# ViennaRNA/RNAcode

Measured on AMD Instinct MI355X. Metric: alignment-columns x samples scored /sec, higher is better.
Workload: dtype f32; 1 GPU; synthetic MAF 10000 blocks x 120 cols x 6 seqs, n=1000 (BASELINE configs[2]/[3]); exchange=none, fit_exp_mode=fused

## Files before the change

### rnacode_amd/csrc/rc_context.cpp

```cpp
#include <cstddef>

#include "rc_runtime.h"

extern "C" {

const char *rc_last_error(void) { return g_err.c_str(); }

void rc_default_params(rc_params *p) {
  p->Delta = -10.0f; p->Omega = -4.0f; p->omega = -2.0f;
  p->stopPenalty_0 = -9999.0f; p->stopPenalty_k = -8.0f;
  p->blosum = 62; p->sampleN = 100; p->cutoff = 1.0f; p->stopEarly = 0; p->seed_base = 42;
  std::memset(p->genetic_code, 0, sizeof p->genetic_code);
}

}

void want_hw_queues() { (void)setenv("GPU_MAX_HW_QUEUES", "8", 0); }

int table_set(rc_ctx *c, const rc_params &par, const TableSet **out) {
  char code[64];
  const char *why = nullptr;
  if (!parse_genetic_code(par.genetic_code, code, &why)) return fail(RC_ERR_ARG, why);
  if (par.blosum != 62 && par.blosum != 90) return fail(RC_ERR_ARG, "blosum must be 62 or 90");
  std::lock_guard<std::mutex> lk(c->setMutex);
// ... 37 lines not shown
  c->sets.push_back(std::move(t));
  return RC_OK;
}

extern "C" {

int rc_device_count(void) {
  want_hw_queues();
  int n = 0;
  if (hipGetDeviceCount(&n) != hipSuccess) return 0;
  return n;
}

int rc_host_cpus(void) { return effective_cpus(); }

void rc_ctx_trim(rc_ctx *c) {
  if (!c) return;
  (void)hipSetDevice(c->device);
  (void)hipDeviceSynchronize();
  c->retired->drain();
  c->bufPool->drain(false);
}

void rc_ctx_destroy(rc_ctx *c) {
  if (!c) return;
  (void)hipSetDevice(c->device);
  (void)hipDeviceSynchronize();
  c->retired->ctxGone.store(true);
  c->retired->drain();
  g_retired.drain();
  c->bufPool->drain(true);
  c->pool.reset();
  if (kProfiling && c->d_cellStats.p) {
    unsigned long long st[8] = {0, 0, 0, 0, 0, 0, 0, 0};
    if (hipMemcpy(st, c->d_cellStats.p, sizeof st, hipMemcpyDeviceToHost) == hipSuccess && st[0])
      std::fprintf(stderr, "[rc cell stats] wavefront-cells %llu, with no positive lane %llu (%.4f %%), positive lane-cells %.2f %%\n", st[0], st[1],
                   100.0 * st[1] / st[0], 100.0 * st[2] / (64.0 * st[0])),
      std::fprintf(stderr, "[rc cell stats] before the row's first event %.1f %%, event codons %.1f %%, after its last event %.1f %%, between events %.1f %%\n",
                   100.0 * st[3] / st[0], 100.0 * st[4] / st[0], 100.0 * st[5] / st[0], 100.0 * (st[0] - st[3] - st[4] - st[5]) / st[0]),
      std::fprintf(stderr, "[rc cell stats] buffered row: chunks tested against the scan's gate %llu, passed over %llu (%.2f %%)\n", st[6], st[7],
                   st[6] ? 100.0 * st[7] / st[6] : 0.0);
  }
  if (c->d_U) (void)hipFree(c->d_U);
  for (hipStream_t st : c->compute) if (st) (void)hipStreamDestroy(st);
  if (c->native) (void)hipStreamDestroy(c->native);
  if (c->copy) (void)hipStreamDestroy(c->copy);
  if (c->aux) (void)hipStreamDestroy(c->aux);
  if (c->tree) (void)hipStreamDestroy(c->tree);
  if (c->tree2) (void)hipStreamDestroy(c->tree2);
  for (hipStream_t st : c->classStreams) (void)hipStreamDestroy(st);
  delete c;
}

int rc_ctx_create(int device, rc_ctx **out) {
  if (!out) return fail(RC_ERR_ARG, "null out pointer");
  *out = nullptr;
  want_hw_queues();
  int n = 0;
  trace("ctx: start", nullptr);
  if (hipGetDeviceCount(&n) != hipSuccess || n <= 0)
    return fail(RC_ERR_DEVICE, "no HIP device available: the scoring path has no CPU fallback");
  trace("ctx: runtime up", nullptr);
  if (device < 0 || device >= n) return fail(RC_ERR_ARG, "device index out of range");
  HIP_TRY(hipSetDevice(device));
  std::unique_ptr<rc_ctx, void (*)(rc_ctx *)> guard(new rc_ctx(), rc_ctx_destroy);
  rc_ctx *c = guard.get();
  c->device = device;
  hipDeviceProp_t prop;
  HIP_TRY(hipGetDeviceProperties(&prop, device));
  c->numCU = prop.multiProcessorCount;
  c->totalMem = prop.totalGlobalMem;
  c->retiredCapBytes = prop.totalGlobalMem / 16;
  c->bufPool->devCap = prop.totalGlobalMem / 16;
  c->bufPool->device = device;
// ... 20 lines not shown
  if (const char *e = std::getenv("RC_DUAL_ROWS")) c->dualRows = std::atoi(e) != 0;
  if (const char *e = std::getenv("RC_HIGH_OCCUPANCY")) c->highOccupancy = std::max(0, std::min(2, std::atoi(e)));
  if (prop.maxSharedMemoryPerMultiProcessor > 0) c->ldsPerCU = prop.maxSharedMemoryPerMultiProcessor;
  if (const char *e = std::getenv("RC_FAT_STREAM_MIN_ITEMS")) c->fatStreamMinItems = std::max(0ll, std::atoll(e));
  if (const char *e = std::getenv("RC_GENERIC_SCRATCH_MB")) c->genericScratchWords = std::max<size_t>(1, static_cast<size_t>(std::atoll(e))) * (1u << 20) / sizeof(uint32_t);
  int prioLow = 0, prioHigh = 0;
  HIP_TRY(hipDeviceGetStreamPriorityRange(&prioLow, &prioHigh));
  c->prioLow = prioLow; c->prioHigh = 0; c->classPrio = prioLow;
  trace("ctx: streams", nullptr);
  c->serialNative = std::getenv("RC_SERIAL_NATIVE") ? 1 : 0;
  c->stopTwoRoundsMinItems = 4LL * c->numCU * 16;
  if (const char *e = std::getenv("RC_STOP_MIN_ITEMS")) c->stopTwoRoundsMinItems = std::atoll(e);
  if (const char *e = std::getenv("RC_GENERIC_MIN_ROWS")) c->rule.genericMinRows = std::max(3, std::min(kTemplRows + 1, std::atoi(e)));
  if (const char *e = std::getenv("RC_TILED_MAX_L")) c->rule.tiledMaxL = std::max(0, std::atoi(e));
  if (const char *e = std::getenv("RC_TILED_MIN_ROWS")) c->rule.tiledMinRows = std::max(kTiledMaxKT + 2, std::min(kTemplRows + 1, std::atoi(e)));
  if (const char *e = std::getenv("RC_TILED_MAX_ROWS")) c->rule.tiledMaxRows = std::max(kTemplRows, std::min(kMaxRows, std::atoi(e)));
  if (const char *e = std::getenv("RC_TILED_WIDE_MAX_L")) c->rule.tiledWideMaxL = std::max(0, std::atoi(e));
  if (const char *e = std::getenv("RC_TILED_ANY_L_MIN_ROWS")) c->rule.tiledAnyLMinRows = std::max(kTemplRows + 1, std::atoi(e));
  if (const char *e = std::getenv("RC_STOP_ROUNDS")) c->stopRounds = std::max(2, std::min(kMaxRounds, std::atoi(e)));
  {
    rc_params std{};
    std.blosum = 62;
    const TableSet *unused = nullptr;
    RC_TRY(table_set(c, std, &unused));
    std.blosum = 90;
    RC_TRY(table_set(c, std, &unused));
  }
  trace("ctx: tables", nullptr);
  c->tieThr = float_threshold_lt(0.0001);
  if (const char *e = std::getenv("RC_LDS_MAX_BYTES")) { c->ldsMaxBytes = c->ldsMaxBytesOneRow = static_cast<size_t>(std::atol(e)); c->stageManyRows = true; }
#ifdef RC_PROFILING
  if (const char *e = std::getenv("RC_DEBUG_SKIP")) c->debugSkip = std::atoi(e);
  if (std::getenv("RC_CELL_STATS")) {
    HIP_TRY(c->d_cellStats.ensure(8 * sizeof(unsigned long long)));
    HIP_TRY(hipMemset(c->d_cellStats.p, 0, 8 * sizeof(unsigned long long)));
  }
#endif
  c->hostThreads = std::min(effective_cpus(), 32);
  if (const char *e = std::getenv("RC_HOST_THREADS")) c->hostThreads = std::max(1, std::atoi(e));
  *out = guard.release();
  return RC_OK;
}

int rc_genetic_code(int32_t ncbi_id, char out[65]) {
  if (!out) return fail(RC_ERR_ARG, "null out pointer");
  const char *aas = ncbi_code(ncbi_id);
  if (!aas) return fail(RC_ERR_ARG, "unknown genetic code id " + std::to_string(ncbi_id) +
                                    " (built in: 1-6, 9-14, 16, 21-26, 29, 30, 33; 27, 28, 31 and 32 are not supported)");
  std::memcpy(out, aas, 64);
  out[64] = '\0';
  return RC_OK;
}

int rc_ctx_set_host_threads(rc_ctx *c, int32_t threads) {
  if (!c || threads < 1) return fail(RC_ERR_ARG, "bad argument");
  if (c->inflight.load() != 0) return fail(RC_ERR_ARG, "batches are in flight");
  c->hostThreads = threads;
  c->pool.reset();
  return RC_OK;
}

int rc_ctx_host_threads(const rc_ctx *c) { return c ? c->hostThreads : 0; }

int rc_ctx_fit_exp_mode(const rc_ctx *c) { return c ? c->expMode : RC_ERR_ARG; }

}

#undef rc_default_params
// ... 33 lines not shown
```

### rnacode_amd/csrc/rc_null_kernel.h

```cpp
#pragma once
#include <hip/hip_runtime.h>

#include <type_traits>
#include <utility>

#include "rc_device.h"
#include "rc_launch.h"
#include "rc_scan_core.h"
#include "rc_sim_core.h"

namespace rc {


template <bool SEM> __device__ __forceinline__ float ref_max(float x, float y) {
  if constexpr (SEM) return x > y ? x : y;
  else return fmaxf(x, y);
}
template <bool SEM> __device__ __forceinline__ float ref_max3(float x, float y, float z) { return ref_max<SEM>(ref_max<SEM>(x, y), z); }

template <bool SEM = false>
__device__ __forceinline__ void pair_step(int zc, float sig, float Delta, float Omega, float omega,
                                          float &s0, float &s1, float &s2) {
  if (zc == 0) {
    s0 = s0 + sig;
// ... 37 lines not shown
      const float v = (j < sites) ? rows[static_cast<size_t>(a - aLo) * sites + j] : 0.0f;
      const bool last = (a == sites - 1) && (j == sites - 1);
      unsigned long long m = __ballot((j < sites) && (v > 0.0f || last));
      while (m) {
        const int t = __builtin_ctzll(m);
        m &= m - 1ull;
        const int jj = j0 + t;
        const float vt = __int_as_float(__builtin_amdgcn_readlane(__float_as_int(v), t));
        scan_step(st, vt, a, jj, (a == sites - 1) && (jj == sites - 1), tieThr, [&](const ScanState &e) {
          if (out && lane == 0 && n < hssCap) out[n] = DevHss{s, f, e.ss, e.se, e.cm};
          n++;
        });
      }
    }
  }
}


template <int K> struct KReg { float s0, s1, s2; int lut; };
template <typename Seq> struct KRegs;
template <int... K> struct KRegs<std::integer_sequence<int, K...>> : KReg<K>... {
  template <int I> __device__ __forceinline__ KReg<I> &at() { return static_cast<KReg<I> &>(*this); }
};
template <int NK, typename F, int... K>
__device__ __forceinline__ void static_for_impl(F &&f, std::integer_sequence<int, K...>) {
  (f(std::integral_constant<int, K>{}), ...);
}
template <int NK, typename F> __device__ __forceinline__ void static_for(F &&f) {
  static_for_impl<NK>(static_cast<F &&>(f), std::make_integer_sequence<int, NK>{});
}

template <int NK, bool EXACT> __device__ __forceinline__ float div_by_nk(float x, float nkf) {
  if constexpr ((NK & (NK - 1)) == 0) {
    return x * (1.0f / static_cast<float>(NK));
  } else if constexpr (EXACT) {
    return x / nkf;
  } else {
    constexpr float y = 1.0f / static_cast<float>(NK);
    const float q0 = x * y;
    const float r = __builtin_fmaf(-static_cast<float>(NK), q0, x);
    return __builtin_fmaf(r, y, q0);
  }
}


struct DeepFetch {};
template <int OFF> struct StagedSite { uint32_t at; };
template <typename T> struct IsStagedSite : std::false_type {};
template <int OFF> struct IsStagedSite<StagedSite<OFF>> : std::true_type {};
template <int OFF> constexpr int staged_off(StagedSite<OFF>) { return OFF; }
__device__ __forceinline__ int site_index(int j) { return j; }
template <int OFF> __device__ __forceinline__ int site_index(StagedSite<OFF>) { return 0; }

template <int NK, bool LDSC, bool EXACT, bool DUAL, int MODE = 0>
__device__ __forceinline__ void null_body(const NullArgs &A, const uint8_t *__restrict__ blob,
                                          const DevBlock *__restrict__ dblocks, const int *__restrict__ classBlocks,
                                          const uint32_t *__restrict__ flags, const uint32_t *__restrict__ Ustream, const uint8_t *__restrict__ pairTab,
                                          uint32_t *__restrict__ scratch, float *__restrict__ maxima) {
  constexpr int N = NK + 1;
  constexpr int CPW = 5;
  constexpr int NCW = (NK + CPW - 1) / CPW;
  constexpr bool kTableLookups = !LDSC && !EXACT;
  constexpr int kTableWords = kTableLookups ? NK * kWave : 0;
  constexpr int LB = code_tail_bytes(NK);
  constexpr int PSW = code_pos_words(NK);
  using TailT = std::conditional_t<LB == 1, uint8_t, std::conditional_t<LB == 2, uint16_t, uint32_t>>;
  constexpr int ZW = (NK + 31) / 32;
  using Regs = KRegs<std::make_integer_sequence<int, NK>>;
  static_assert(!DUAL || (!EXACT && NK <= kDualRowsMaxNK), "two rows per pass: fast division, few sequences");
  static_assert(!(LDSC && EXACT), "the EXACT instantiation uses no LDS");
  constexpr bool ROWS = MODE == 1, SIM = MODE == 2;
#ifndef RC_DEEP_FETCH_MAX_NK
#define RC_DEEP_FETCH_MAX_NK 31
#endif
// ... 333 lines not shown
                  }
                }
                if (w < NCW - 1) {
                  store_words(std::integral_constant<int, 4>{}, laneWord, wf, wr, siteF + w * kWave * 4, siteR + w * kWave * 4);
                } else {
                  store_words(std::integral_constant<int, LB>{}, laneTailB, wf, wr, siteF + (NCW - 1) * kWave * 4, siteR + (NCW - 1) * kWave * 4);
                }
              }
            }
          }
        }
      }
      if (clamped && (kLean ? lane == 0 : sidx < A.sampleN) && (SIM || onlyCombo <= 0)) atomicAdd(A.clampCount, static_cast<unsigned long long>(clamped));
    }
    if constexpr (SIM) continue;
    if (!helping && shared) {
      const size_t G = gridDim.x;
      if (lane == 0) {
        __hip_atomic_store(A.steal + kStealHdr + G + 2 * blockIdx.x, static_cast<unsigned int>(bi), __ATOMIC_RELAXED, __HIP_MEMORY_SCOPE_AGENT);
        __hip_atomic_store(A.steal + kStealHdr + G + 2 * blockIdx.x + 1, static_cast<unsigned int>(grp), __ATOMIC_RELAXED, __HIP_MEMORY_SCOPE_AGENT);
      }
      __builtin_amdgcn_fence(__ATOMIC_RELEASE, "agent");
      __builtin_amdgcn_s_waitcnt(0);
      if (lane == 0) {
        atomicExch(A.steal + kStealHdr + blockIdx.x, 1u);
        const unsigned int idx = atomicAdd(A.steal, 1u);
        __hip_atomic_store(A.steal + kStealHdr + 3 * G + idx, (blockIdx.x + 1u) | (static_cast<unsigned int>(home) << 24), __ATOMIC_RELAXED, __HIP_MEMORY_SCOPE_AGENT);
        atomicSub(A.steal + 1, 1u);
      }
      firstCombo = claim_part(slot);
    }

    float best = -1.0f;
    unsigned long long statCells = 0, statNoPos = 0, statPosLanes = 0, statPristine = 0, statEvent = 0, statTail = 0, statGateTested = 0, statGateSkipped = 0;
    float omega_v, Delta_v = 0.0f;
    asm volatile("v_mov_b32 %0, %1" : "=v"(omega_v) : "s"(omega));
    float rcpNk_v = 0.0f, negNk_v = 0.0f;
    if constexpr (!EXACT && (NK & (NK - 1)) != 0) {
      asm volatile("v_mov_b32 %0, %1" : "=v"(rcpNk_v) : "s"(1.0f / static_cast<float>(NK)));
      asm volatile("v_mov_b32 %0, %1" : "=v"(negNk_v) : "s"(-static_cast<float>(NK)));
    }
    if constexpr (EXACT) asm volatile("v_mov_b32 %0, %1" : "=v"(Delta_v) : "s"(Delta));
    if (!kProfiling || !(A.debugSkip & 1)) {
      Regs R;
      int curS = -1;
      for (int c = onlyCombo >= 0 ? onlyCombo : firstCombo; c < 6; c = onlyCombo >= 0 ? 6 : (shared ? claim_part(slot) : c + 1)) {
        const int s = c >= 3 ? 1 : 0, f = c - 3 * s;
        if (s != curS) {
          static_for<NK>([&](auto kc) {
            constexpr int k = decltype(kc)::value;
            R.template at<k>().lut = __float_as_int(lut[(s * NK + k) * kLutSize + lane]);
            if constexpr (kTableLookups) lds_codes[k * kWave + lane] = static_cast<uint32_t>(R.template at<k>().lut);
          });
          curS = s;
        }
        const int sites = (L - f) / 3;
        if (sites <= 0) continue;
        const uint32_t *__restrict__ sbase = cod + static_cast<size_t>(s * L1 + 3 + f) * PSW;
        constexpr int kSiteWords = 3 * PSW;
        auto word_at = [&](int j, int x) -> uint32_t {
          const uint32_t *p = sbase + static_cast<size_t>(j) * kSiteWords;
          if (x < NCW - 1) return p[x * kWave + lane];
          return static_cast<uint32_t>(reinterpret_cast<const TailT *>(p + (NCW - 1) * kWave)[lane]);
        };
        const unsigned long long *__restrict__ zbase = zw + static_cast<size_t>(s * L1 + 3 + f) * ZW;
        const unsigned long long *__restrict__ zany = zmask + static_cast<size_t>(s * 3 + f) * zmWords;
        int jc = sites;
// ... 122 lines not shown
          auto wait_lookups = [&](auto leave) {
            constexpr int k0 = (NCW - 1) * CPW;
            constexpr int cnt = NK - k0;
            constexpr int left = (decltype(leave)::value > 0 && !decltype(scalarLoadsNearby)::value) ? decltype(leave)::value : 0;
            if constexpr (cnt == 1) asm volatile("s_waitcnt lgkmcnt(%1)" : "+v"(sig[k0]) : "n"(left));
            else if constexpr (cnt == 2) asm volatile("s_waitcnt lgkmcnt(%2)" : "+v"(sig[k0]), "+v"(sig[k0 + 1]) : "n"(left));
            else if constexpr (cnt == 3) asm volatile("s_waitcnt lgkmcnt(%3)" : "+v"(sig[k0]), "+v"(sig[k0 + 1]), "+v"(sig[k0 + 2]) : "n"(left));
            else if constexpr (cnt == 4)
              asm volatile("s_waitcnt lgkmcnt(%4)" : "+v"(sig[k0]), "+v"(sig[k0 + 1]), "+v"(sig[k0 + 2]), "+v"(sig[k0 + 3]) : "n"(left));
            else
              asm volatile("s_waitcnt lgkmcnt(%5)" : "+v"(sig[k0]), "+v"(sig[k0 + 1]), "+v"(sig[k0 + 2]), "+v"(sig[k0 + 3]), "+v"(sig[k0 + 4]) : "n"(left));
            static_for<NK>([&](auto kc) {
              constexpr int k = decltype(kc)::value;
              if constexpr (k < k0) {
                float b = sig[k];
                asm volatile("" : "+v"(b), "+v"(sig[k0]));
                sig[k] = b;
              }
            });
          };
          if constexpr (LDSC) {
            if constexpr (IsStagedSite<std::decay_t<decltype(jn)>>::value) fetch_staged_at(w, jn);
            else fetch_staged(w, jn);
            wait_lookups(std::integral_constant<int, NCW>{});
          } else if constexpr (!EXACT) {
            if constexpr (std::is_same_v<std::decay_t<decltype(kind)>, DeepFetch>) fetch_global(w, pnext);
            else if (jn >= jc) fetch_cached(w, jn);
            else fetch_global(w, pnext);
            wait_lookups(std::integral_constant<int, 0>{});
          } else {
            wait_lookups(std::integral_constant<int, 0>{});
          }
        };
        auto finish = [&](float sum) -> float {
          if constexpr (kProfiling) {
            const unsigned long long pos = __ballot(sum > 0.0f);
            statCells++; statNoPos += (pos == 0ull); statPosLanes += __builtin_popcountll(pos);
          }
          if constexpr (EXACT) {
            const float top = (sum > Delta_v) ? sum : Delta_v;
            return div_by_nk<NK, EXACT>(top, nkf);
          } else {
            if constexpr ((NK & (NK - 1)) == 0) return div_by_nk<NK, EXACT>(sum, nkf);
            else {
              const float q0 = sum * rcpNk_v;
              const float r = __builtin_fmaf(negNk_v, q0, sum);
              return __builtin_fmaf(r, rcpNk_v, q0);
            }
          }
        };
        auto fast_cell = [&](uint32_t (&w)[NCW], int jn, auto kind) -> float {
          float sig[NK];
          lookup(w, sig, jn, std::false_type{}, kind);
          float sum = 0.0f;
          static_for<NK>([&](auto kc) {
            constexpr int k = decltype(kc)::value;
            auto &r = R.template at<k>();
            r.s0 = r.s0 + sig[k];
            r.s1 = r.s1 + omega_v;
            r.s2 = r.s2 + omega_v;
            const float m = fmaxf(fmaxf(r.s0, r.s1), r.s2);
            sum = (k == 0) ? m : sum + m;
          });
          return finish(sum);
        };
        auto pristine_cell = [&](uint32_t (&w)[NCW], float &wv, int jn, auto kind) -> float {
          float sig[NK];
          lookup(w, sig, jn, std::false_type{}, kind);
          wv = wv + omega_v;
          float sum = 0.0f;
          static_for<NK>([&](auto kc) {
            constexpr int k = decltype(kc)::value;
            auto &r = R.template at<k>();
            r.s0 = r.s0 + sig[k];
            const float m = fmaxf(r.s0, wv);
            sum = (k == 0) ? m : sum + m;
          });
          return finish(sum);
        };
        auto tail_cell = [&](uint32_t (&w)[NCW], int jn, auto kind) -> float {
          float sig[NK];
          lookup(w, sig, jn, std::false_type{}, kind);
// ... 32 lines not shown
            j = (j | 63) + 1;
          }
          return end;
        };
        SampleScan st{0.0f, 0.0f, 0u, 0u};
        float negTwo_v;
        asm volatile("v_mov_b32 %0, -2.0" : "=v"(negTwo_v));
        const float negTie = -A.tieThr;
        auto deep_pairs = [&](int &j, uint32_t (&wcur)[NCW], int e, auto &&act) {
          const int lim = e < jc - 2 ? e : jc - 2;
          if (lim - j >= 4) {
            uint32_t wB[NCW];
            {
              const uint32_t *p = sbase + static_cast<size_t>(j + 1) * kSiteWords;
              asm volatile("s_nop 4" : "+s"(p));
              fetch_global(wB, p);
            }
            for (; j + 2 <= lim; j += 2) {
              act(wcur, j, j + 2);
              act(wB, j + 1, j + 3);
            }
#pragma unroll
            for (int x = 0; x < NCW; x++) asm volatile("s_waitcnt vmcnt(0)" : "+v"(wB[x]));
          }
        };
        if constexpr (DUAL) {
          typedef float RowBuf __attribute__((ext_vector_type(32)));
          constexpr int kBuf = 32;
          constexpr int kGroup = 4;
          constexpr int kGateChunk = 4;
          static_assert(kGateChunk >= 2 && kBuf % kGateChunk == 0, "whole chunks fill the buffer");
          RowBuf buf = {};
          Regs RB;
          auto pristine2 = [&](uint32_t (&w)[NCW], float &wvA, float &wvB, auto jn, float &vB, auto kd) -> float {
            float sig[NK];
            lookup(w, sig, jn, std::false_type{}, kd);
            wvA = wvA + omega_v;
            wvB = wvB + omega_v;
            float sumA = 0.0f, sumB = 0.0f;
            static_for<NK>([&](auto kc) {
              constexpr int k = decltype(kc)::value;
              auto &ra = R.template at<k>();
              auto &rb = RB.template at<k>();
              ra.s0 = ra.s0 + sig[k];
              const float ma = fmaxf(ra.s0, wvA);
              sumA = (k == 0) ? ma : sumA + ma;
              rb.s0 = rb.s0 + sig[k];
              const float mb = fmaxf(rb.s0, wvB);
              sumB = (k == 0) ? mb : sumB + mb;
            });
            vB = finish(sumB);
            return finish(sumA);
          };
          auto fast2 = [&](uint32_t (&w)[NCW], auto jn, float &vB, auto kd) -> float {
            float sig[NK];
            lookup(w, sig, jn, std::false_type{}, kd);
            float sumA = 0.0f, sumB = 0.0f;
            static_for<NK>([&](auto kc) {
              constexpr int k = decltype(kc)::value;
              auto &ra = R.template at<k>();
              auto &rb = RB.template at<k>();
              ra.s0 = ra.s0 + sig[k];
              ra.s1 = ra.s1 + omega_v;
              ra.s2 = ra.s2 + omega_v;
              const float ma = fmaxf(fmaxf(ra.s0, ra.s1), ra.s2);
              sumA = (k == 0) ? ma : sumA + ma;
              rb.s0 = rb.s0 + sig[k];
              rb.s1 = rb.s1 + omega_v;
              rb.s2 = rb.s2 + omega_v;
              const float mb = fmaxf(fmaxf(rb.s0, rb.s1), rb.s2);
              sumB = (k == 0) ? mb : sumB + mb;
            });
            vB = finish(sumB);
            return finish(sumA);
          };
          auto tail2 = [&](uint32_t (&w)[NCW], auto jn, float &vB, auto kd) -> float {
            float sig[NK];
            lookup(w, sig, jn, std::false_type{}, kd);
            float sumA = 0.0f, sumB = 0.0f;
            static_for<NK>([&](auto kc) {
              constexpr int k = decltype(kc)::value;
              auto &ra = R.template at<k>();
              auto &rb = RB.template at<k>();
              ra.s0 = ra.s0 + sig[k];
              ra.s1 = ra.s1 + omega_v;
              const float ma = fmaxf(ra.s0, ra.s1);
              sumA = (k == 0) ? ma : sumA + ma;
              rb.s0 = rb.s0 + sig[k];
              rb.s1 = rb.s1 + omega_v;
              const float mb = fmaxf(rb.s0, rb.s1);
              sumB = (k == 0) ? mb : sumB + mb;
            });
            vB = finish(sumB);
            return finish(sumA);
          };
          auto event2 = [&](uint32_t (&w)[NCW], int j, int jn, float &vB) -> float {
            float sig[NK];
            lookup(w, sig, jn, std::true_type{}, std::true_type{});
            unsigned long long z[ZW];
#pragma unroll
            for (int x = 0; x < ZW; x++) z[x] = zbase[static_cast<size_t>(3 * j) * ZW + x];
            float sumA = 0.0f, sumB = 0.0f;
            static_for<NK>([&](auto kc) {
              constexpr int k = decltype(kc)::value;
              auto &ra = R.template at<k>();
              auto &rb = RB.template at<k>();
              const int zc = static_cast<int>((z[k >> 5] >> (2 * (k & 31))) & 3ull);
              pair_step(zc, sig[k], Delta, Omega, omega, ra.s0, ra.s1, ra.s2);
              const float ma = fmaxf(fmaxf(ra.s0, ra.s1), ra.s2);
              sumA = (k == 0) ? ma : sumA + ma;
              pair_step(zc, sig[k], Delta, Omega, omega, rb.s0, rb.s1, rb.s2);
              const float mb = fmaxf(fmaxf(rb.s0, rb.s1), rb.s2);
              sumB = (k == 0) ? mb : sumB + mb;
            });
            vB = finish(sumB);
            return finish(sumA);
          };
          int a = 0;
          int pendRow = -1, pendExtra = 0, pendN = 0;
          while (a < sites || pendRow >= 0) {
            if (pendRow < 0 && a + 2 < sites && !((zany[a >> 6] >> (a & 63)) & 1ull)) {
              sample_scan_row_begin(st, best, static_cast<uint32_t>(a));
              static_for<NK>([&](auto kc) {
                constexpr int k = decltype(kc)::value;
                auto &r = R.template at<k>();
                r.s0 = r.s1 = r.s2 = 0.0f;
                auto &rb = RB.template at<k>();
                rb.s0 = rb.s1 = rb.s2 = 0.0f;
              });
              uint32_t wcur[NCW];
              load_words(a, wcur);
              int j = a;
              float wvA = 0.0f, wvB = 0.0f;
              asm volatile("v_mov_b32 %0, 0" : "=v"(wvA));
              asm volatile("v_mov_b32 %0, 0" : "=v"(wvB));
              {
                const float v = pristine_cell(wcur, wvA, a + 1, std::true_type{});
                sample_scan_step(st, v, negTie, negTwo_v);
                j = a + 1;
              }
              const int extra = (sites - 1 - a > kBuf) ? sites - 1 - a - kBuf : 0;
              const int b0 = a + 1 + extra;
              auto keep = [&](float vB, int jj) {
                const int idx = jj > b0 ? jj - b0 : 0;
                buf[idx] = vB;
              };
              auto pair_cell = [&](uint32_t (&w)[NCW], int jj, int jn, auto kd, auto &&fn) {
                float vB;
                const float v = fn(w, jn, vB, kd);
                sample_scan_step(st, v, negTie, negTwo_v);
                keep(vB, jj);
              };
              auto dspan = [&](int e, auto &&fn) {
                if constexpr (!LDSC && !EXACT && MODE == 0)
                  deep_pairs(j, wcur, e, [&](uint32_t (&w)[NCW], int jj, int jn) { pair_cell(w, jj, jn, DeepFetch{}, fn); });
                if constexpr (LDSC) {
                  for (const int pe = e < b0 ? e : b0; j < pe; j++) {
                    float vB;
                    const float v = fn(wcur, j + 1, vB, std::true_type{});
                    sample_scan_step(st, v, negTie, negTwo_v);
                  }
                  const int ge = e < sites - 1 ? e : sites - 1;
                  for (; j + kGroup <= ge; j += kGroup) {
                    const uint32_t at = ldsLane + static_cast<uint32_t>(j + 1) * (NCW * kWave * 4u);
                    float vB[kGroup];
                    static_for<kGroup>([&](auto uc) {
                      constexpr int u = decltype(uc)::value;
                      const float v = fn(wcur, StagedSite<u * NCW * kWave * 4>{at}, vB[u], std::true_type{});
                      sample_scan_step(st, v, negTie, negTwo_v);
                    });
                    int idxRaw = j - b0;
                    asm volatile("" : "+s"(idxRaw));
                    const int idx = idxRaw & (kBuf - 1);
                    __builtin_amdgcn_sched_barrier(0);
                    static_for<kGroup>([&](auto uc) {
                      constexpr int u = decltype(uc)::value;
                      buf[idx + u] = vB[u];
                    });
                    __builtin_amdgcn_sched_barrier(0);
                  }
                }
                for (; j < e; j++) pair_cell(wcur, j, j + 1 < sites ? j + 1 : j, std::true_type{}, fn);
              };
              {
                if constexpr (kProfiling) statPristine += 1 + 2 * (next_event(j, sites) - j);
                dspan(next_event(j, sites), [&](uint32_t (&w)[NCW], auto jn, float &vB, auto kd) { return pristine2(w, wvA, wvB, jn, vB, kd); });
                static_for<NK>([&](auto kc) {
                  constexpr int k = decltype(kc)::value;
                  auto &r = R.template at<k>();
                  r.s1 = r.s2 = wvA;
                  auto &rb = RB.template at<k>();
                  rb.s1 = rb.s2 = wvB;
                });
              }
              while (j < sites) {
                if ((zany[j >> 6] >> (j & 63)) & 1ull) {
                  const int jev = j;
                  if constexpr (kProfiling) statEvent += 2;
                  pair_cell(wcur, j, j + 1 < sites ? j + 1 : j, std::true_type{}, [&](uint32_t (&w)[NCW], int jn, float &vB, auto) { return event2(w, jev, jn, vB); });
                  j++;
                }
                const int e = next_event(j, sites);
                if (e == sites) {
                  static_for<NK>([&](auto kc) {
                    constexpr int k = decltype(kc)::value;
                    auto &r = R.template at<k>();
                    r.s1 = fmaxf(r.s1, r.s2);
                    auto &rb = RB.template at<k>();
                    rb.s1 = fmaxf(rb.s1, rb.s2);
                  });
                  if constexpr (kProfiling) statTail += 2 * (e - j);
                  dspan(e, [&](uint32_t (&w)[NCW], auto jn, float &vB, auto kd) { return tail2(w, jn, vB, kd); });
// ... 35 lines not shown
                  constexpr int k = decltype(kc)::value;
                  auto &r = R.template at<k>();
                  r.s1 = r.s2 = wv;
                });
              }
              while (j < jend) {
                if ((zany[j >> 6] >> (j & 63)) & 1ull) {
                  if constexpr (kProfiling) statEvent++;
                  const int jj = j;
                  one([&](uint32_t (&w)[NCW], int jn, auto kd) { return event_cell(w, jj, jn, kd, std::false_type{}); });
                  j++;
                }
                const int e = next_event(j, jend);
                if (e == jend) {
                  static_for<NK>([&](auto kc) {
                    constexpr int k = decltype(kc)::value;
                    auto &r = R.template at<k>();
                    r.s1 = fmaxf(r.s1, r.s2);
                  });
                  for (; j < e; j++) one([&](uint32_t (&w)[NCW], int jn, auto kd) {
                    if constexpr (kProfiling) statTail++;
                    return tail_cell(w, jn, kd);
                  });
                }
                for (; j < e; j++) one([&](uint32_t (&w)[NCW], int jn, auto kd) { return fast_cell(w, jn, kd); });
              }
#pragma unroll
              for (int x = 0; x < NCW; x++) {
                if constexpr (LDSC) asm volatile("s_waitcnt lgkmcnt(0)" : "+v"(wcur[x]));
                else asm volatile("s_waitcnt vmcnt(0) lgkmcnt(0)" : "+v"(wcur[x]));
              }
              if (pend) {
                if constexpr (!EXACT) {
                  float G = sample_scan_gate(st, best, negTie);
                  [&]() {
#pragma unroll
                    for (int c0 = 0; c0 < kBuf; c0 += kGateChunk) {
                      if (c0 + kGateChunk > pendN) {
#pragma unroll
                        for (int u = 0; u < kGateChunk - 1; u++) {
                          if (c0 + u >= pendN) return;
                          sample_scan_step(st, buf[c0 + u], negTie, negTwo_v);
                        }
                        return;
                      }
                      float m = buf[c0];
#pragma unroll
                      for (int u = 1; u + 1 < kGateChunk; u += 2) m = scan_max3(m, buf[c0 + u], buf[c0 + u + 1]);
                      if constexpr (kGateChunk % 2 == 0) m = scan_max(m, buf[c0 + kGateChunk - 1]);
                      if constexpr (kProfiling) statGateTested++;
                      if (__builtin_amdgcn_ballot_w64(sample_scan_gate_pass(m, G)) != 0ull) {
#pragma unroll
                        for (int u = 0; u < kGateChunk; u++) sample_scan_step(st, buf[c0 + u], negTie, negTwo_v);
                        G = sample_scan_gate(st, best, negTie);
                      } else {
                        if constexpr (kProfiling) statGateSkipped++;
                        sample_scan_skip(st, kGateChunk);
                      }
                    }
                  }();
                } else {
                  [&]() {
#pragma unroll
                    for (int idx = 0; idx < kBuf; idx++) {
                      if (idx >= pendN) return;
                      sample_scan_step(st, buf[idx], negTie, negTwo_v);
                    }
                  }();
                }
                pendRow = -1;
              } else {
                a += 1;
              }
              sample_scan_row_end(st, static_cast<uint32_t>(row), static_cast<uint32_t>(row == sites - 1 ? sites - 1 : sites));
            }
          }
        } else {
          int aLo = 0, aHi = sites;
          float *sdst = nullptr;
          if constexpr (ROWS) {
            const long long total = static_cast<long long>(sites) * (sites + 1) / 2;
            auto row_at = [&](long long cellsBefore) {
              int a = 0;
              long long cum = 0;
              while (a < sites && cum < cellsBefore) { cum += sites - a; a++; }
              return a;
            };
            aLo = row_at(total * rowPart / rowParts);
            aHi = rowPart + 1 == rowParts ? sites : row_at(total * (rowPart + 1) / rowParts);
            const long long before = static_cast<long long>(aLo) * sites - static_cast<long long>(aLo) * (aLo - 1) / 2;
            sdst = A.sbuf + (static_cast<size_t>(itemIndex) * 6 + c) * A.sbufStride + static_cast<size_t>(before) * kWave + lane;
          }
          for (int a = aLo; a < aHi; a++) {
            if constexpr (!ROWS) sample_scan_row_begin(st, best, static_cast<uint32_t>(a));
            static_for<NK>([&](auto kc) {
              constexpr int k = decltype(kc)::value;
              auto &r = R.template at<k>();
              r.s0 = r.s1 = r.s2 = 0.0f;
            });
// ... 50 lines not shown
              const int e = next_event(j, jend);
              if (e == jend) {
                static_for<NK>([&](auto kc) {
                  constexpr int k = decltype(kc)::value;
                  auto &r = R.template at<k>();
                  r.s1 = fmaxf(r.s1, r.s2);
                });
                span(e, [&](uint32_t (&w)[NCW], int jn, auto kd) {
                  if constexpr (kProfiling) statTail++;
                  return tail_cell(w, jn, kd);
                });
              }
              span(e, [&](uint32_t (&w)[NCW], int jn, auto kd) { return fast_cell(w, jn, kd); });
            }
            if constexpr (!EXACT) {
#pragma unroll
              for (int x = 0; x < NCW; x++) {
                if constexpr (LDSC) asm volatile("s_waitcnt lgkmcnt(0)" : "+v"(wcur[x]));
                else asm volatile("s_waitcnt vmcnt(0) lgkmcnt(0)" : "+v"(wcur[x]));
              }
            }
            if constexpr (ROWS) { if (a == sites - 1) sdst += kWave; }
            else sample_scan_row_end(st, static_cast<uint32_t>(a), static_cast<uint32_t>(jend));
          }
        }
        if constexpr (!ROWS) sample_scan_last(st, best);
      }
    }
    if constexpr (kProfiling) {
      if (A.cellStats && lane == 0) {
        atomicAdd(A.cellStats, statCells); atomicAdd(A.cellStats + 1, statNoPos); atomicAdd(A.cellStats + 2, statPosLanes);
        atomicAdd(A.cellStats + 3, statPristine); atomicAdd(A.cellStats + 4, statEvent); atomicAdd(A.cellStats + 5, statTail);
        atomicAdd(A.cellStats + 6, statGateTested); atomicAdd(A.cellStats + 7, statGateSkipped);
      }
    }
    if (!ROWS && sidx < A.sampleN) {
      float *dst = maxima + static_cast<size_t>(db->out_index) * A.sampleN + sidx;
      if (A.comboSplit || shared) { if (best > -1.0f) atomicMax(reinterpret_cast<int *>(dst), __float_as_int(best)); }
      else *dst = best;
    }
  }
}

constexpr int null_min_waves(int NK, bool EXACT, bool DUAL, int MODE) { return DUAL ? (NK == 2 && MODE == 0 ? 5 : 4) :(EXACT || MODE != 0) ? 1 : NK == 6 ? 6 : (NK == 9 || NK == 10) ? 5 : (NK >= 16 && NK <= 21) ? 4 : (NK >= 24 && NK <= 29) ? 3 : 1; }
template <int NK, bool LDSC, bool EXACT, bool DUAL = false, int MODE = 0>
__global__ __launch_bounds__(64) __attribute__((amdgpu_waves_per_eu(null_min_waves(NK, EXACT, DUAL, MODE))))
void k_null(NullArgs A, const uint8_t *__restrict__ blob,
                                             const DevBlock *__restrict__ dblocks, const int *__restrict__ classBlocks,
                                             const uint32_t *__restrict__ flags, const uint32_t *__restrict__ Ustream, const uint8_t *__restrict__ pairTab,
                                             uint32_t *__restrict__ scratch, float *__restrict__ maxima) {
  null_body<NK, LDSC, EXACT, DUAL, MODE>(A, blob, dblocks, classBlocks, flags, Ustream, pairTab, scratch, maxima);
}

constexpr int hi_occ_waves(int NK) { return (NK >= 6 && NK <= 8) ? 6 : (NK >= 10 && NK <= 12) ? 5 : 0; }
template <int NK>
__global__ __launch_bounds__(64) __attribute__((amdgpu_waves_per_eu(hi_occ_waves(NK) ? hi_occ_waves(NK) : 1)))
void k_null_occ(NullArgs A, const uint8_t *__restrict__ blob, const DevBlock *__restrict__ dblocks, const int *__restrict__ classBlocks,
                const uint32_t *__restrict__ flags, const uint32_t *__restrict__ Ustream, const uint8_t *__restrict__ pairTab,
                uint32_t *__restrict__ scratch, float *__restrict__ maxima) {
  null_body<NK, false, false, false>(A, blob, dblocks, classBlocks, flags, Ustream, pairTab, scratch, maxima);
}


template <int NK>
inline int null_occupancy_one(NullKind kind, size_t lds) {
  int nb = 0;
// ... 61 lines not shown
```

### rnacode_amd/csrc/rc_scan_core.h

```cpp
#pragma once
#include <cmath>
#include <cstdint>

#if defined(__HIPCC__)
#define RC_SCAN_D __device__ __forceinline__
#else
#define RC_SCAN_D inline
#endif

namespace rc {

struct SampleScan {
  float cm;
  float X;
  uint32_t se;
  uint32_t len;
};

RC_SCAN_D float scan_med3(float a, float b, float c) {
#if defined(__HIP_DEVICE_COMPILE__)
  return __builtin_amdgcn_fmed3f(a, b, c);
#else
  const float lo = a < b ? a : b, hi = a < b ? b : a;
  return c < lo ? lo : (c > hi ? hi : c);
// ... 32 lines not shown
  const uint32_t j = jn + static_cast<uint32_t>((x >> 1) + 1);
  st.se = inrow ? j : st.se;
  st.len = j - a;
}
RC_SCAN_D void sample_scan_last(const SampleScan &st, float &best) {
  best = ((st.len >= 2u) & (st.cm > best)) ? st.cm : best;
}

RC_SCAN_D float scan_max(float a, float b) {
#if defined(__HIP_DEVICE_COMPILE__)
  float r;
  asm("v_max_f32 %0, %1, %2" : "=v"(r) : "v"(a), "v"(b));
  return r;
#else
  return fmaxf(a, b);
#endif
}
RC_SCAN_D float scan_max3(float a, float b, float c) {
#if defined(__HIP_DEVICE_COMPILE__)
  float r;
  asm("v_max3_f32 %0, %1, %2, %3" : "=v"(r) : "v"(a), "v"(b), "v"(c));
  return r;
#else
  return fmaxf(fmaxf(a, b), c);
#endif
}
RC_SCAN_D float sample_scan_gate(const SampleScan &st, float best, float negTieThr) {
  const float c = scan_max(st.cm, best);
  return scan_med3(0.0f, c + 2.0f * negTieThr, c * 0.99999976158142089844f);
}
RC_SCAN_D bool sample_scan_gate_pass(float m, float G) { return m > G; }
RC_SCAN_D void sample_scan_skip(SampleScan &st, int n) { st.X = st.X + static_cast<float>(-2 * n); }

}
```

Measured before the change: 30.70 billion alignment-columns*samples/s.

## Gate row-a groups and buffered row on undivided sums, deferring the division

The buffered row and row-a scan now store raw column sums and divide by NK only when a value actually enters the scan step. Row a's staged groups of four are now tested against a gate rescaled to sum units, so whole groups whose maximum cannot update any lane skip the per-cell scan steps and divisions. Ballot-driven early exit replays the group only when some lane needs it. The scaled gate has a small rounding margin, and the extra ballot and control flow could cost more than they save when groups rarely skip.

```diff
diff --git a/rnacode_amd/csrc/rc_context.cpp b/rnacode_amd/csrc/rc_context.cpp
--- a/rnacode_amd/csrc/rc_context.cpp
+++ b/rnacode_amd/csrc/rc_context.cpp
@@ -93,14 +93,16 @@
   c->bufPool->drain(true);
   c->pool.reset();
   if (kProfiling && c->d_cellStats.p) {
-    unsigned long long st[8] = {0, 0, 0, 0, 0, 0, 0, 0};
+    unsigned long long st[10] = {0, 0, 0, 0, 0, 0, 0, 0, 0, 0};
     if (hipMemcpy(st, c->d_cellStats.p, sizeof st, hipMemcpyDeviceToHost) == hipSuccess && st[0])
       std::fprintf(stderr, "[rc cell stats] wavefront-cells %llu, with no positive lane %llu (%.4f %%), positive lane-cells %.2f %%\n", st[0], st[1],
                    100.0 * st[1] / st[0], 100.0 * st[2] / (64.0 * st[0])),
       std::fprintf(stderr, "[rc cell stats] before the row's first event %.1f %%, event codons %.1f %%, after its last event %.1f %%, between events %.1f %%\n",
                    100.0 * st[3] / st[0], 100.0 * st[4] / st[0], 100.0 * st[5] / st[0], 100.0 * (st[0] - st[3] - st[4] - st[5]) / st[0]),
       std::fprintf(stderr, "[rc cell stats] buffered row: chunks tested against the scan's gate %llu, passed over %llu (%.2f %%)\n", st[6], st[7],
-                   st[6] ? 100.0 * st[7] / st[6] : 0.0);
+                   st[6] ? 100.0 * st[7] / st[6] : 0.0),
+      std::fprintf(stderr, "[rc cell stats] row a: groups of four tested against the gate on sums %llu, passed over %llu (%.2f %%)\n", st[8], st[9],
+                   st[8] ? 100.0 * st[9] / st[8] : 0.0);
   }
   if (c->d_U) (void)hipFree(c->d_U);
   for (hipStream_t st : c->compute) if (st) (void)hipStreamDestroy(st);
@@ -187,8 +189,8 @@
 #ifdef RC_PROFILING
   if (const char *e = std::getenv("RC_DEBUG_SKIP")) c->debugSkip = std::atoi(e);
   if (std::getenv("RC_CELL_STATS")) {
-    HIP_TRY(c->d_cellStats.ensure(8 * sizeof(unsigned long long)));
-    HIP_TRY(hipMemset(c->d_cellStats.p, 0, 8 * sizeof(unsigned long long)));
+    HIP_TRY(c->d_cellStats.ensure(10 * sizeof(unsigned long long)));
+    HIP_TRY(hipMemset(c->d_cellStats.p, 0, 10 * sizeof(unsigned long long)));
   }
 #endif
   c->hostThreads = std::min(effective_cpus(), 32);
diff --git a/rnacode_amd/csrc/rc_null_kernel.h b/rnacode_amd/csrc/rc_null_kernel.h
--- a/rnacode_amd/csrc/rc_null_kernel.h
+++ b/rnacode_amd/csrc/rc_null_kernel.h
@@ -93,14 +93,11 @@
 
 template <int NK, bool EXACT> __device__ __forceinline__ float div_by_nk(float x, float nkf) {
   if constexpr ((NK & (NK - 1)) == 0) {
-    return x * (1.0f / static_cast<float>(NK));
+    return scan_div_nk(x, 1.0f / static_cast<float>(NK), -static_cast<float>(NK), true);
   } else if constexpr (EXACT) {
     return x / nkf;
   } else {
-    constexpr float y = 1.0f / static_cast<float>(NK);
-    const float q0 = x * y;
-    const float r = __builtin_fmaf(-static_cast<float>(NK), q0, x);
-    return __builtin_fmaf(r, y, q0);
+    return scan_div_nk(x, 1.0f / static_cast<float>(NK), -static_cast<float>(NK), false);
   }
 }
 
@@ -500,7 +497,7 @@
     }
 
     float best = -1.0f;
-    unsigned long long statCells = 0, statNoPos = 0, statPosLanes = 0, statPristine = 0, statEvent = 0, statTail = 0, statGateTested = 0, statGateSkipped = 0;
+    unsigned long long statCells = 0, statNoPos = 0, statPosLanes = 0, statPristine = 0, statEvent = 0, statTail = 0, statGateTested = 0, statGateSkipped = 0, statGroupTested = 0, statGroupSkipped = 0;
     float omega_v, Delta_v = 0.0f;
     asm volatile("v_mov_b32 %0, %1" : "=v"(omega_v) : "s"(omega));
     float rcpNk_v = 0.0f, negNk_v = 0.0f;
@@ -689,22 +686,24 @@
             wait_lookups(std::integral_constant<int, 0>{});
           }
         };
-        auto finish = [&](float sum) -> float {
+        auto seen = [&](float sum) {
           if constexpr (kProfiling) {
             const unsigned long long pos = __ballot(sum > 0.0f);
             statCells++; statNoPos += (pos == 0ull); statPosLanes += __builtin_popcountll(pos);
           }
+        };
+        auto divide = [&](float sum) -> float {
           if constexpr (EXACT) {
             const float top = (sum > Delta_v) ? sum : Delta_v;
             return div_by_nk<NK, EXACT>(top, nkf);
           } else {
             if constexpr ((NK & (NK - 1)) == 0) return div_by_nk<NK, EXACT>(sum, nkf);
-            else {
-              const float q0 = sum * rcpNk_v;
-              const float r = __builtin_fmaf(negNk_v, q0, sum);
-              return __builtin_fmaf(r, rcpNk_v, q0);
-            }
-          }
+            else return scan_div_nk(sum, rcpNk_v, negNk_v, false);
+          }
+        };
+        auto finish = [&](float sum) -> float {
+          seen(sum);
+          return divide(sum);
         };
         auto fast_cell = [&](uint32_t (&w)[NCW], int jn, auto kind) -> float {
           float sig[NK];
@@ -803,6 +802,7 @@
           static_assert(kGateChunk >= 2 && kBuf % kGateChunk == 0, "whole chunks fill the buffer");
           RowBuf buf = {};
           Regs RB;
+          constexpr float kNkF = static_cast<float>(NK);
           auto pristine2 = [&](uint32_t (&w)[NCW], float &wvA, float &wvB, auto jn, float &vB, auto kd) -> float {
             float sig[NK];
             lookup(w, sig, jn, std::false_type{}, kd);
@@ -820,8 +820,10 @@
               const float mb = fmaxf(rb.s0, wvB);
               sumB = (k == 0) ? mb : sumB + mb;
             });
-            vB = finish(sumB);
-            return finish(sumA);
+            seen(sumB);
+            seen(sumA);
+            vB = sumB;
+            return sumA;
           };
           auto fast2 = [&](uint32_t (&w)[NCW], auto jn, float &vB, auto kd) -> float {
             float sig[NK];
@@ -842,8 +844,10 @@
               const float mb = fmaxf(fmaxf(rb.s0, rb.s1), rb.s2);
               sumB = (k == 0) ? mb : sumB + mb;
             });
-            vB = finish(sumB);
-            return finish(sumA);
+            seen(sumB);
+            seen(sumA);
+            vB = sumB;
+            return sumA;
           };
           auto tail2 = [&](uint32_t (&w)[NCW], auto jn, float &vB, auto kd) -> float {
             float sig[NK];
@@ -862,8 +866,10 @@
               const float mb = fmaxf(rb.s0, rb.s1);
               sumB = (k == 0) ? mb : sumB + mb;
             });
-            vB = finish(sumB);
-            return finish(sumA);
+            seen(sumB);
+            seen(sumA);
+            vB = sumB;
+            return sumA;
           };
           auto event2 = [&](uint32_t (&w)[NCW], int j, int jn, float &vB) -> float {
             float sig[NK];
@@ -884,8 +890,10 @@
               const float mb = fmaxf(fmaxf(rb.s0, rb.s1), rb.s2);
               sumB = (k == 0) ? mb : sumB + mb;
             });
-            vB = finish(sumB);
-            return finish(sumA);
+            seen(sumB);
+            seen(sumA);
+            vB = sumB;
+            return sumA;
           };
           int a = 0;
           int pendRow = -1, pendExtra = 0, pendN = 0;
@@ -912,43 +920,65 @@
               }
               const int extra = (sites - 1 - a > kBuf) ? sites - 1 - a - kBuf : 0;
               const int b0 = a + 1 + extra;
-              auto keep = [&](float vB, int jj) {
+              auto keep = [&](float sB, int jj) {
                 const int idx = jj > b0 ? jj - b0 : 0;
-                buf[idx] = vB;
+                buf[idx] = sB;
               };
               auto pair_cell = [&](uint32_t (&w)[NCW], int jj, int jn, auto kd, auto &&fn) {
-                float vB;
-                const float v = fn(w, jn, vB, kd);
+                float sB;
+                const float v = divide(fn(w, jn, sB, kd));
                 sample_scan_step(st, v, negTie, negTwo_v);
-                keep(vB, jj);
+                keep(sB, jj);
               };
               auto dspan = [&](int e, auto &&fn) {
                 if constexpr (!LDSC && !EXACT && MODE == 0)
                   deep_pairs(j, wcur, e, [&](uint32_t (&w)[NCW], int jj, int jn) { pair_cell(w, jj, jn, DeepFetch{}, fn); });
                 if constexpr (LDSC) {
                   for (const int pe = e < b0 ? e : b0; j < pe; j++) {
-                    float vB;
-                    const float v = fn(wcur, j + 1, vB, std::true_type{});
+                    float sB;
+                    const float v = divide(fn(wcur, j + 1, sB, std::true_type{}));
                     sample_scan_step(st, v, negTie, negTwo_v);
                   }
                   const int ge = e < sites - 1 ? e : sites - 1;
-                  for (; j + kGroup <= ge; j += kGroup) {
-                    const uint32_t at = ldsLane + static_cast<uint32_t>(j + 1) * (NCW * kWave * 4u);
-                    float vB[kGroup];
-                    static_for<kGroup>([&](auto uc) {
-                      constexpr int u = decltype(uc)::value;
-                      const float v = fn(wcur, StagedSite<u * NCW * kWave * 4>{at}, vB[u], std::true_type{});
-                      sample_scan_step(st, v, negTie, negTwo_v);
-                    });
-                    int idxRaw = j - b0;
-                    asm volatile("" : "+s"(idxRaw));
-                    const int idx = idxRaw & (kBuf - 1);
-                    __builtin_amdgcn_sched_barrier(0);
-                    static_for<kGroup>([&](auto uc) {
-                      constexpr int u = decltype(uc)::value;
-                      buf[idx + u] = vB[u];
-                    });
-                    __builtin_amdgcn_sched_barrier(0);
+                  static_assert(kGroup == 4, "a group's maximum: v_max3 + v_max");
+                  float sA[kGroup] = {};
+                  unsigned long long need = 0ull;
+                  asm volatile("" : "+s"(need));
+                  for (;;) {
+                    if (j + kGroup <= ge) {
+                      unsigned long long stop;
+                      do {
+                        const uint32_t at = ldsLane + static_cast<uint32_t>(j + 1) * (NCW * kWave * 4u);
+                        float vB[kGroup];
+                        static_for<kGroup>([&](auto uc) {
+                          constexpr int u = decltype(uc)::value;
+                          sA[u] = fn(wcur, StagedSite<u * NCW * kWave * 4>{at}, vB[u], std::true_type{});
+                        });
+                        int idxRaw = j - b0;
+                        asm volatile("" : "+s"(idxRaw));
+                        const int idx = idxRaw & (kBuf - 1);
+                        __builtin_amdgcn_sched_barrier(0);
+                        static_for<kGroup>([&](auto uc) {
+                          constexpr int u = decltype(uc)::value;
+                          buf[idx + u] = vB[u];
+                        });
+                        __builtin_amdgcn_sched_barrier(0);
+                        const float m = scan_max(scan_max3(sA[0], sA[1], sA[2]), sA[3]);
+                        const float Gs = sample_scan_gate_sum(st, best, negTie, kNkF);
+                        sample_scan_skip(st, kGroup);
+                        j += kGroup;
+                        need = __builtin_amdgcn_ballot_w64(sample_scan_gate_pass(m, Gs));
+                        if constexpr (kProfiling) { statGroupTested++; statGroupSkipped += (need == 0ull); }
+                        const unsigned long long last = static_cast<unsigned long long>(static_cast<long long>(ge - kGroup - j) >> 63);
+                        stop = need | last;
+                      } while (stop == 0ull);
+                    }
+                    if (need == 0ull) break;
+                    need = 0ull;
+                    asm volatile("" : "+s"(need));
+                    sample_scan_skip(st, -kGroup);
+#pragma unroll
+                    for (int u = 0; u < kGroup; u++) sample_scan_step(st, divide(sA[u]), negTie, negTwo_v);
                   }
                 }
                 for (; j < e; j++) pair_cell(wcur, j, j + 1 < sites ? j + 1 : j, std::true_type{}, fn);
@@ -1050,7 +1080,7 @@
               }
               if (pend) {
                 if constexpr (!EXACT) {
-                  float G = sample_scan_gate(st, best, negTie);
+                  float G = sample_scan_gate_sum(st, best, negTie, kNkF);
                   [&]() {
 #pragma unroll
                     for (int c0 = 0; c0 < kBuf; c0 += kGateChunk) {
@@ -1058,7 +1088,7 @@
 #pragma unroll
                         for (int u = 0; u < kGateChunk - 1; u++) {
                           if (c0 + u >= pendN) return;
-                          sample_scan_step(st, buf[c0 + u], negTie, negTwo_v);
+                          sample_scan_step(st, divide(buf[c0 + u]), negTie, negTwo_v);
                         }
                         return;
                       }
@@ -1069,8 +1099,8 @@
                       if constexpr (kProfiling) statGateTested++;
                       if (__builtin_amdgcn_ballot_w64(sample_scan_gate_pass(m, G)) != 0ull) {
 #pragma unroll
-                        for (int u = 0; u < kGateChunk; u++) sample_scan_step(st, buf[c0 + u], negTie, negTwo_v);
-                        G = sample_scan_gate(st, best, negTie);
+                        for (int u = 0; u < kGateChunk; u++) sample_scan_step(st, divide(buf[c0 + u]), negTie, negTwo_v);
+                        G = sample_scan_gate_sum(st, best, negTie, kNkF);
                       } else {
                         if constexpr (kProfiling) statGateSkipped++;
                         sample_scan_skip(st, kGateChunk);
@@ -1082,7 +1112,7 @@
 #pragma unroll
                     for (int idx = 0; idx < kBuf; idx++) {
                       if (idx >= pendN) return;
-                      sample_scan_step(st, buf[idx], negTie, negTwo_v);
+                      sample_scan_step(st, divide(buf[idx]), negTie, negTwo_v);
                     }
                   }();
                 }
@@ -1199,6 +1229,7 @@
         atomicAdd(A.cellStats, statCells); atomicAdd(A.cellStats + 1, statNoPos); atomicAdd(A.cellStats + 2, statPosLanes);
         atomicAdd(A.cellStats + 3, statPristine); atomicAdd(A.cellStats + 4, statEvent); atomicAdd(A.cellStats + 5, statTail);
         atomicAdd(A.cellStats + 6, statGateTested); atomicAdd(A.cellStats + 7, statGateSkipped);
+        atomicAdd(A.cellStats + 8, statGroupTested); atomicAdd(A.cellStats + 9, statGroupSkipped);
       }
     }
     if (!ROWS && sidx < A.sampleN) {
diff --git a/rnacode_amd/csrc/rc_scan_core.h b/rnacode_amd/csrc/rc_scan_core.h
--- a/rnacode_amd/csrc/rc_scan_core.h
+++ b/rnacode_amd/csrc/rc_scan_core.h
@@ -88,4 +88,15 @@
 RC_SCAN_D bool sample_scan_gate_pass(float m, float G) { return m > G; }
 RC_SCAN_D void sample_scan_skip(SampleScan &st, int n) { st.X = st.X + static_cast<float>(-2 * n); }
 
+RC_SCAN_D float scan_div_nk(float x, float rcpNk, float negNk, bool pow2) {
+  const float q0 = x * rcpNk;
+  if (pow2) return q0;
+  const float r = __builtin_fmaf(negNk, q0, x);
+  return __builtin_fmaf(r, rcpNk, q0);
 }
+RC_SCAN_D float scan_gate_sum_of(float G, float nk) { return (G * nk) * 0.99999976158142089844f; }
+RC_SCAN_D float sample_scan_gate_sum(const SampleScan &st, float best, float negTieThr, float nk) {
+  return scan_gate_sum_of(sample_scan_gate(st, best, negTieThr), nk);
+}
+
+}
```

Result: faster. 31.13 billion alignment-columns*samples/s (median of 6 runs) (+1.4%).
